# mcychan/nQuant.android

Measured on NVIDIA B200. Metric: Mpixels/s 256-color PNN quantize+dither, 4K batch, 1/2/4/8 B200 vs JVM CPU, higher is better.
Workload: dtype f64

## Files before the change

### include/nquant_b200.h

```cpp
#ifndef NQUANT_B200_H
#define NQUANT_B200_H

#include <stdint.h>

#ifdef __cplusplus
extern "C" {
#endif

#define NQ_KIND_PNN 0
#define NQ_KIND_PNNLAB 1

#define NQ_OK 0
#define NQ_ERR_CUDA (-1)
#define NQ_ERR_ARG (-2)
#define NQ_ERR_COLOR (-3)
#define NQ_ERR_UNSUPPORTED (-4)
#define NQ_ERR_NOMEM (-5)

typedef struct nq_ctx nq_ctx;

int nq_device_count(void);

nq_ctx* nq_create(int device);
void nq_destroy(nq_ctx* ctx);
// ... 24 lines not shown
                           int dither, uint64_t rng_seed, const uint32_t* palette_in, int palette_len, uint32_t* argb_out);

int nq_histogram(nq_ctx* ctx, int kind, const uint32_t* argb_in, int width, int height, int n_max_colors, int* n_bins,
                 double* bins5, float* init_err, int* init_nn, int capacity);

int nq_gilbert_order(int width, int height, uint32_t* order_out);


typedef struct nq_image_info {
  int has_semi_transparency;
  int transparent_pixel_index;
  uint32_t transparent_color;
  int maxbins, quan_rt, texicab, is_nano;
  double weight, ratio_init, ratio_merge, pr, pg, pb, pa;
  int g_margin, g_thresold, g_dither_max_q, g_dither_max, g_sorted, g_has_alpha, g_use_saliency;
  float g_beta;
  float bn_weight;
  int palette_len;
  unsigned long long merges, rescans, pair_tests, rng_draws, heap_pops;
  int error;
  unsigned long long full_evals;
  unsigned long long merge_cycles[6], live_blocks, screened;
  unsigned long long dither_cycles[3];
} nq_image_info;
int nq_get_image_info(nq_ctx* ctx, int image, nq_image_info* out);
int nq_sizeof_image_info(void);

int nq_set_spec_dither(nq_ctx* ctx, int on, int segment, int warmup);
int nq_get_spec_stats(nq_ctx* ctx, unsigned long long* images, unsigned long long* rounds, unsigned long long* fallbacks);

int nq_set_debug(nq_ctx* ctx, int flag);
int nq_debug_get_bins(nq_ctx* ctx, int image, double* bins5, float* init_err, int* init_nn);
int nq_debug_get_merges(nq_ctx* ctx, int image, int* pairs);
int nq_debug_get_saliencies(nq_ctx* ctx, int image, float* out);

unsigned long long nq_kernel_launches(nq_ctx* ctx);
int nq_get_stage_times(nq_ctx* ctx, double* ms, unsigned long long* launches, int reset);
int nq_get_kernel_times(nq_ctx* ctx, double* ms, unsigned long long* launches, int reset);
int nq_debug_math(nq_ctx* ctx, int fn, const double* x, const double* y, double* out, int n);

int nq_debug_ciede(nq_ctx* ctx, const float* lab1, const float* lab2, float* out, int* n_exact, int n);

int nq_synth_device(nq_ctx* ctx, uint32_t* d_out, int n_images, int width, int height, int cls, int alpha_mode,
                    uint64_t seed0);

#ifdef __cplusplus
// ... 4 lines not shown
```

### nquant_android_b200/_lib.py

```python
import ctypes
import os

HERE = os.path.dirname(os.path.abspath(__file__))
SO = os.path.join(HERE, "libnquant_b200.so")

SYMBOLS = [
    "nq_device_count", "nq_create", "nq_destroy", "nq_last_error", "nq_convert", "nq_convert_batch",
    "nq_convert_batch_device", "nq_dither_with_palette", "nq_gilbert_order", "nq_get_image_info", "nq_set_debug",
    "nq_debug_get_bins", "nq_debug_get_merges", "nq_debug_get_saliencies", "nq_kernel_launches", "nq_debug_math",
    "nq_synth_device", "nq_get_stage_times", "nq_set_stream", "nq_debug_ciede", "nq_sizeof_image_info",
    "nq_set_spec_dither", "nq_get_spec_stats", "nq_reset_stream", "nq_set_chunk_images", "nq_get_kernel_times", "nq_convert_batch_multi", "nq_histogram",
]

NQ_KIND_PNN, NQ_KIND_PNNLAB = 0, 1
NQ_OK, NQ_ERR_CUDA, NQ_ERR_ARG, NQ_ERR_COLOR, NQ_ERR_UNSUPPORTED, NQ_ERR_NOMEM = 0, -1, -2, -3, -4, -5


class ImageInfo(ctypes.Structure):
    _fields_ = [
        ("has_semi_transparency", ctypes.c_int), ("transparent_pixel_index", ctypes.c_int),
        ("transparent_color", ctypes.c_uint32),
        ("maxbins", ctypes.c_int), ("quan_rt", ctypes.c_int), ("texicab", ctypes.c_int), ("is_nano", ctypes.c_int),
        ("weight", ctypes.c_double), ("ratio_init", ctypes.c_double), ("ratio_merge", ctypes.c_double),
        ("pr", ctypes.c_double), ("pg", ctypes.c_double), ("pb", ctypes.c_double), ("pa", ctypes.c_double),
        ("g_margin", ctypes.c_int), ("g_thresold", ctypes.c_int), ("g_dither_max_q", ctypes.c_int),
        ("g_dither_max", ctypes.c_int), ("g_sorted", ctypes.c_int), ("g_has_alpha", ctypes.c_int),
        ("g_use_saliency", ctypes.c_int),
        ("g_beta", ctypes.c_float), ("bn_weight", ctypes.c_float), ("palette_len", ctypes.c_int),
        ("merges", ctypes.c_ulonglong), ("rescans", ctypes.c_ulonglong), ("pair_tests", ctypes.c_ulonglong),
        ("rng_draws", ctypes.c_ulonglong), ("heap_pops", ctypes.c_ulonglong),
        ("error", ctypes.c_int),
        ("full_evals", ctypes.c_ulonglong),
        ("merge_cycles", ctypes.c_ulonglong * 6), ("live_blocks", ctypes.c_ulonglong), ("screened", ctypes.c_ulonglong),
        ("dither_cycles", ctypes.c_ulonglong * 3),
    ]

    def as_dict(self):
        return {n: (list(getattr(self, n)) if n in ("merge_cycles", "dither_cycles") else getattr(self, n)) for n, _ in self._fields_}


_lib = None


def load():
    global _lib
    if _lib is not None:
        return _lib
    if not os.path.exists(SO):
        raise ImportError(f"{SO} is missing: run `python -c 'import __graft_entry__ as g; g.build()'` "
                          "(nvcc, sm_100a). This package has no CPU fallback.")
    L = ctypes.CDLL(SO)
    vp, ci, u64 = ctypes.c_void_p, ctypes.c_int, ctypes.c_uint64
    L.nq_device_count.restype = ci
    L.nq_create.restype = vp
    L.nq_create.argtypes = [ci]
    L.nq_destroy.argtypes = [vp]
    L.nq_destroy.restype = None
# ... 32 lines not shown
```

### nquant_android_b200/csrc/nq_api.cu

```cuda
#include <cuda_runtime.h>
#include <stdint.h>
#include <stdio.h>
#include <stdlib.h>
#include <string.h>
#include <string>
#include <vector>
#include <map>
#include <utility>
#include <algorithm>
#include <mutex>
#include <thread>
#include <atomic>
#include <nvtx3/nvToolsExt.h>

#include "../../include/nquant_b200.h"
#include "nq_types.h"
#include "nq_math.h"
#include "nq_color.h"
#include "nq_bluenoise_table.h"
#include "nq_hist.cuh"
#include "nq_pnn.cuh"
#include "nq_dither.cuh"
#include "nq_dither_spec.cuh"

// ... 129 lines not shown
  std::vector<double> bins5;
  std::vector<float> initErr;
  std::vector<int> initNn;
  std::vector<int> merges;
  std::vector<float> sal;
};

}

#define NQ_FRONT_STREAMS 2
#define NQ_SPEC_BULK_DEFAULT 0

struct nq_ctx {
  int device = 0;
  cudaStream_t stream = nullptr;
  cudaStream_t ownStream = nullptr;
  cudaStream_t sFront[NQ_FRONT_STREAMS] = {}, sDith = nullptr, sAux = nullptr, sOut = nullptr, sIn = nullptr;
  std::vector<cudaEvent_t> evPool;
  size_t evUsed = 0;
  int smCount = 148;
  unsigned long long launches = 0;
  bool debug = false;
  int chunkImages = 0;
  int mergeRot = 0;
  std::map<std::pair<int, int>, uint32_t*> orders;
  std::vector<std::pair<int, int>> orderLru;
  size_t orderBytes = 0;
  unsigned char* ws = nullptr;
  size_t wsBytes = 0;
  NqImage* dImgs = nullptr;
  NqSlot* dSlots = nullptr;
  int* dLive = nullptr;
  int* dPos = nullptr;
  unsigned char* zeroPlane = nullptr;
  unsigned char* memoPlane = nullptr;
  unsigned char* sortPool = nullptr;
  size_t zeroSlotBytes = 0, memoSlotBytes = 0, sortSetBytes = 0, sortABytes = 0;
  int wsSlots = 0, wsNpix = 0, wsKind = -1, sortSets = 0;
  bool wsDebug = false, wsBits = false, wsIdx = false;
  std::vector<NqSlot> hSlots;
  uint32_t* dIn = nullptr;
  uint32_t* dOut = nullptr;
  size_t stageBytes = 0;
  double stageMs[NQ_NSTAGES] = {};
  unsigned long long stageLaunches[NQ_NSTAGES] = {};
  double kernelMs[NQ_NKERNELS] = {};
  unsigned long long kernelLaunches[NQ_NKERNELS] = {};
// ... 403 lines not shown
        std::vector<double> col(mb);
        std::vector<float> colf(mb);
        for (int k = 0; k < 4; ++k) {
          if (kind == NQ_KIND_RGB) {
            const double* src = k == 0 ? S.bAc : k == 1 ? S.bC1 : k == 2 ? S.bC2 : S.bC3;
            CU(cudaMemcpy(col.data(), src, (size_t)mb * 8, cudaMemcpyDeviceToHost));
          } else {
            const float* src = k == 0 ? S.fAc : k == 1 ? S.fC1 : k == 2 ? S.fC2 : S.fC3;
            CU(cudaMemcpy(colf.data(), src, (size_t)mb * 4, cudaMemcpyDeviceToHost));
            for (int b = 0; b < mb; ++b) col[b] = colf[b];
          }
          for (int b = 0; b < mb; ++b) D.bins5[(size_t)b * 5 + k] = col[b];
        }
        CU(cudaMemcpy(colf.data(), S.bCnt, (size_t)mb * 4, cudaMemcpyDeviceToHost));
        for (int b = 0; b < mb; ++b) D.bins5[(size_t)b * 5 + 4] = colf[b];
        CU(cudaMemcpy(D.initErr.data(), S.bErr, (size_t)mb * 4, cudaMemcpyDeviceToHost));
        CU(cudaMemcpy(D.initNn.data(), S.bNn, (size_t)mb * 4, cudaMemcpyDeviceToHost));
      }
    }
    if (A.stopAfterSweep) { mark(4); CU(cudaGetLastError()); return NQ_OK; }
    int* live = c->dLive + (size_t)ch.base * NQ_NBINS;
    int* pos = c->dPos + (size_t)ch.base * NQ_NBINS;
    if (kind == NQ_KIND_RGB) {
      nq::k_merge_rgb<<<n, NQ_RGB_THREADS, (size_t)NQ_RGB_HEAP_SMEM * 8, st>>>(dI, dS, live, pos, c->debug ? 1 : 0, c->mergeRot); ++c->launches;
    } else {
      nq::k_merge_lab<<<n, NQ_LAB_THREADS, (size_t)NQ_LAB_HEAP_SMEM * 8, st>>>(dI, dS, live, pos, c->debug ? 1 : 0, c->mergeRot); ++c->launches;
    }
  } else { mark(2); mark(3); }
  mark(4);
  CU(cudaGetLastError());
  return NQ_OK;
}

int run_dither(nq_ctx* c, Chunk& ch, const GroupArgs& A, const uint32_t* dOrder) {
  NvtxRange nv("nq dither (setup, Gilbert pass, BlueNoise pass)");
  const int n = ch.n, npix = A.w * A.h, kind = A.kind;
  cudaStream_t st = c->sDith, ax = c->sAux;
  NqImage* dI = c->dImgs + ch.base;
  NqSlot* dS = c->dSlots + ch.base;
  unsigned long long l0 = c->launches;
  CU(cudaStreamWaitEvent(st, ch.ev[4], 0));
  CU(cudaEventRecord(ch.evD[0], st));
  nq::k_dither_setup<<<(n + 63) / 64, 64, 0, st>>>(dI, dS, n); ++c->launches;
  if (A.dPalIn) {
    for (int i = 0; i < n; ++i) { k_set_palette<<<1, 256, 0, st>>>(dI, i, A.dPalIn, A.palInLen); ++c->launches; }
    nq::k_dither_setup<<<(n + 63) / 64, 64, 0, st>>>(dI, dS, n); ++c->launches;
  }
  const dim3 pg(pixel_grid_x(c, npix, n), n);
  if (kind == NQ_KIND_LAB && c->debug) { nq::k_saliency<<<pg, 256, 0, st>>>(dI, dS); ++c->launches; }
// ... 260 lines not shown
  if (device < 0 || device >= n) { fail(NQ_ERR_CUDA, "no such CUDA device (this library has no CPU fallback)"); return nullptr; }
  if (cudaSetDevice(device) != cudaSuccess) { fail(NQ_ERR_CUDA, "cudaSetDevice failed"); return nullptr; }
  nq_ctx* c = new nq_ctx();
  c->device = device;
  cudaDeviceProp prop;
  if (cudaGetDeviceProperties(&prop, device) == cudaSuccess) c->smCount = prop.multiProcessorCount;
  bool ok = cudaStreamCreateWithFlags(&c->ownStream, cudaStreamNonBlocking) == cudaSuccess;
  for (int k = 0; ok && k < NQ_FRONT_STREAMS; ++k) ok = cudaStreamCreateWithFlags(&c->sFront[k], cudaStreamNonBlocking) == cudaSuccess;
  ok = ok && cudaStreamCreateWithFlags(&c->sDith, cudaStreamNonBlocking) == cudaSuccess;
  ok = ok && cudaStreamCreateWithFlags(&c->sAux, cudaStreamNonBlocking) == cudaSuccess;
  ok = ok && cudaStreamCreateWithFlags(&c->sOut, cudaStreamNonBlocking) == cudaSuccess;
  ok = ok && cudaStreamCreateWithFlags(&c->sIn, cudaStreamNonBlocking) == cudaSuccess;
  if (!ok) { fail(NQ_ERR_CUDA, "cudaStreamCreate failed"); destroy_ctx(c, false); return nullptr; }
  c->stream = c->ownStream;
  if (const char* e = getenv("NQ_SPEC_DITHER")) c->specDither = atoi(e) != 0;
  if (const char* e = getenv("NQ_CHUNK")) c->chunkImages = atoi(e);
  {
    const char* e = getenv("NQ_SPEC_BULK");
    const int bulk = e ? (atoi(e) != 0) : NQ_SPEC_BULK_DEFAULT;
    ok = ok && cudaMemcpyToSymbol(nq::spec::g_specBulk, &bulk, sizeof(bulk)) == cudaSuccess;
  }
  if (const char* e = getenv("NQ_SPEC_SLOTS")) c->specSlotsMax = atoi(e);
  if (const char* e = getenv("NQ_SPEC_POOL_GB")) c->specPoolMaxBytes = (size_t)atoi(e) << 30;
  if (const char* e = getenv("NQ_MERGE_ROT")) c->mergeRot = atoi(e) != 0;
  bool haveLut = false;
  {
    DevBuf dBn, dW;
    ok = dBn.alloc(4096) == cudaSuccess && cudaMemcpy(dBn.p, kBlueNoise, 4096, cudaMemcpyHostToDevice) == cudaSuccess &&
         dW.alloc(sizeof(float) * 3 * (NQ_MAXQ + 3)) == cudaSuccess && cudaMalloc(&c->dTanh, sizeof(float) * 512) == cudaSuccess;
    if (ok) {
      nq::k_init_tables<<<4, 256, 0, c->stream>>>(dBn.as<signed char>()); ++c->launches;
      nq::k_init_rtfac<<<1, 256, 0, c->stream>>>(); ++c->launches;
      k_spec_tables<<<2, 256, 0, c->stream>>>(c->dTanh, dW.as<float>()); ++c->launches;
      ok = cudaMemcpyToSymbolAsync(nq::spec::c_specW, dW.p, sizeof(float) * 3 * (NQ_MAXQ + 3), 0, cudaMemcpyDeviceToDevice, c->stream) == cudaSuccess &&
           cudaStreamSynchronize(c->stream) == cudaSuccess;
    }
  }
  if (ok) {
    std::lock_guard<std::mutex> lk(g_lutMutex);
    LabLutEntry& e = g_lut[device];
    if (!e.ptr) {
      ok = cudaMalloc(&e.ptr, sizeof(float4) << 24) == cudaSuccess;
      if (ok) {
        nq::k_build_lab_lut<<<65536, 256, 0, c->stream>>>(e.ptr); ++c->launches;
        const float4* cp = e.ptr;
        ok = cudaMemcpyToSymbolAsync(nq::g_labLut, &cp, sizeof(cp), 0, cudaMemcpyHostToDevice, c->stream) == cudaSuccess &&
             cudaStreamSynchronize(c->stream) == cudaSuccess;
// ... 128 lines not shown
int nq_gilbert_order(int w, int h, uint32_t* out) {
  if (w <= 0 || h <= 0 || !out) return fail(NQ_ERR_ARG, "bad arguments");
  size_t n = 0;
  gilbert_walk(w, h, [&](int x, int y) { out[n++] = (uint32_t)(x + y * w); });
  return n == (size_t)w * h ? NQ_OK : fail(NQ_ERR_ARG, "gilbert walk size mismatch");
}

int nq_get_image_info(nq_ctx* c, int image, nq_image_info* o) {
  if (!c || !o || image < 0 || image >= (int)c->lastImgs.size()) return fail(NQ_ERR_ARG, "no such image in the last batch");
  const NqImage& I = c->lastImgs[image];
  memset(o, 0, sizeof(*o));
  o->has_semi_transparency = I.hasSemi; o->transparent_pixel_index = I.transIdx; o->transparent_color = I.transColor;
  o->maxbins = I.maxbins; o->quan_rt = I.quan_rt; o->texicab = I.texicab; o->is_nano = I.isNano;
  o->weight = I.weight; o->ratio_init = I.ratio; o->ratio_merge = I.ratioMerge;
  o->pr = I.PR; o->pg = I.PG; o->pb = I.PB; o->pa = I.PA;
  o->g_margin = I.gMargin; o->g_thresold = I.gThresold; o->g_dither_max_q = I.gDitherMaxQ; o->g_dither_max = I.gDitherMax;
  o->g_sorted = I.gSorted; o->g_has_alpha = I.gHasAlpha; o->g_use_saliency = I.gUseSal; o->g_beta = I.gBeta;
  o->bn_weight = I.bnWeight; o->palette_len = I.paletteLen;
  o->merges = (I.nmax > 2 && I.extbins > 0) ? (unsigned long long)I.extbins : 0ULL;
  o->rescans = I.statRescans; o->pair_tests = I.statPairs; o->rng_draws = I.rngDraws; o->heap_pops = I.statHeapPops;
  o->full_evals = I.statFullEvals;
  for (int k = 0; k < 6; ++k) o->merge_cycles[k] = I.statCyc[k];
  o->live_blocks = I.statLiveBlocks; o->screened = I.statScreened;
  for (int k = 0; k < 3; ++k) o->dither_cycles[k] = I.statDither[k];
  o->error = I.error;
  return NQ_OK;
}

int nq_sizeof_image_info(void) { return (int)sizeof(nq_image_info); }

int nq_set_stream(nq_ctx* c, void* stream) {
  if (!c) return fail(NQ_ERR_ARG, "null context");
  c->stream = stream ? reinterpret_cast<cudaStream_t>(stream) : cudaStreamLegacy;
  return NQ_OK;
}
int nq_reset_stream(nq_ctx* c) {
  if (!c) return fail(NQ_ERR_ARG, "null context");
  c->stream = c->ownStream;
  return NQ_OK;
}
int nq_set_chunk_images(nq_ctx* c, int images) {
  if (!c || images < 0) return fail(NQ_ERR_ARG, "bad arguments");
  c->chunkImages = images;
  return NQ_OK;
}

// ... 110 lines not shown
```

### nquant_android_b200/csrc/nq_pnn.cuh

```cuda
#pragma once
#include "nq_types.h"
#include "nq_color.h"
#include "nq_hist.cuh"
#include "nq_fastmath.cuh"

namespace nq {

__device__ const float c_coeffs[3][3] = {{0.299f, 0.587f, 0.114f}, {-0.14713f, -0.28886f, 0.436f}, {0.615f, -0.51499f, -0.10001f}};

struct RgbProbe {
  float n1;
  double wa, wr, wg, wb;
  double PR, PG, PB, PA, ratio;
  int start;
  bool semi;
};

__device__ __forceinline__ RgbProbe rgb_probe(const NqImage& I, const NqSlot& S, int idx) {
  RgbProbe P;
  P.n1 = S.bCnt[idx];
  P.wa = S.bAc[idx]; P.wr = S.bC1[idx]; P.wg = S.bC2[idx]; P.wb = S.bC3[idx];
  P.PR = I.PR; P.PG = I.PG; P.PB = I.PB; P.PA = I.PA; P.ratio = I.ratio;
  P.semi = I.hasSemi != 0;
  P.start = 0;
// ... 351 lines not shown
  __device__ __forceinline__ void sift_down(unsigned idnn1, float e1, int heapN) {
    int l = 1, l2;
    for (; (l2 = l + l) <= heapN; l = l2) {
      float ea, eb = 0.f;
      unsigned ia, ib = 0u;
      if (l2 < HS) {
        ea = sErr[l2]; ia = sIdNn[l2];
        if (l2 < heapN) { eb = sErr[l2 + 1]; ib = sIdNn[l2 + 1]; }
      } else {
        const uint4 ch = *reinterpret_cast<const uint4*>(&gH[l2]);
        ea = __uint_as_float(ch.x); ia = ch.y; eb = __uint_as_float(ch.z); ib = ch.w;
      }
      if (l2 < heapN && ea > eb) { ++l2; ea = eb; ia = ib; }
      if (e1 <= ea) break;
      set(l, ia, ea);
    }
    set(l, idnn1, e1);
  }
};
__device__ __forceinline__ unsigned pack_idnn(int id, int nn) { return (unsigned)id | ((unsigned)nn << 16); }

#define NQ_LAB_THREADS 128
#define NQ_LAB_HEAP_SMEM 5632

__device__ __forceinline__ int block_excl_scan_128(int v, int* total, int* sScan ) {
  const unsigned lane = lane_id(), w = threadIdx.x >> 5;
  int x = v;
#pragma unroll
  for (int o = 1; o < 32; o <<= 1) {
    int y = __shfl_up_sync(0xffffffffu, x, o);
    if (lane >= (unsigned)o) x += y;
  }
  if (lane == 31) sScan[w] = x;
  __syncthreads();
  int base = 0, tot = 0;
#pragma unroll
  for (int k = 0; k < NQ_LAB_THREADS / 32; ++k) { const int c = sScan[k]; if (k < (int)w) base += c; tot += c; }
  *total = tot;
  __syncthreads();
  return base + x - v;
}

__device__ __forceinline__ int rebuild_live_lab(const NqSlot& S, const LabScratch& X, int maxbins, int* live, int* posOf, int* sScan) {
  const int t = threadIdx.x;
  const unsigned lane = lane_id(), w = t >> 5;
  const int W = NQ_LAB_THREADS / 32;
// ... 2 lines not shown
  int c = 0;
  for (int b = b0 + (int)lane; b < b1; b += 32) c += S.bMtm[b] != NQ_DELETED;
  int total, j = block_excl_scan_128(c, &total, sScan);
  j = __shfl_sync(0xffffffffu, j, 0);
  for (int base = b0; base < b1; base += 32) {
    const int b = base + (int)lane;
    const bool alive = b < b1 && S.bMtm[b] != NQ_DELETED;
    const unsigned m = __ballot_sync(0xffffffffu, alive);
    if (alive) {
      const int p = j + __popc(m & ((1u << lane) - 1u));
      live[p] = b; posOf[b] = p;
      X.q[p] = make_float4(S.bCnt[b], S.fC1[b], S.fC2[b], S.fC3[b]);
      X.al[p] = S.fAc[b];
    }
    j += __popc(m);
  }
  __syncthreads();
  const int nblk = (total + 31) >> 5;
  for (int blk = t; blk < nblk; blk += NQ_LAB_THREADS) lab_block_summary(X.q, total, blk, X.bs);
  __syncthreads();
  return total;
}

__global__ void __launch_bounds__(NQ_LAB_THREADS, 4) k_merge_lab(NqImage* imgs, const NqSlot* slots, int* liveBuf, int* posBuf, int logMerges, int rot) {
  extern __shared__ unsigned char smemRaw[];
  float* sErr = reinterpret_cast<float*>(smemRaw);
  unsigned* sId = reinterpret_cast<unsigned*>(smemRaw + (size_t)NQ_LAB_HEAP_SMEM * 4);
  __shared__ int sScan[8];
  __shared__ unsigned sBits[64];
  __shared__ unsigned short sBlk[2048];
  __shared__ unsigned sMaskA[32];
  __shared__ unsigned sMaskB[32];
  __shared__ int sOffA[33], sOffB[33];
  __shared__ double sGs[NQ_LAB_THREADS], sGw[NQ_LAB_THREADS], sF[NQ_LAB_THREADS];
  __shared__ int sPos[NQ_LAB_THREADS];
  __shared__ double sErrCur;
  __shared__ int sNnCur, sAction, sB1, sHeapN, sIter, sNLive;

  const int img = blockIdx.x;
  NqImage& I = imgs[img];
  if (I.kind != NQ_KIND_LAB || I.nmax <= 2 || I.skipPnn) return;
  const NqSlot& S = slots[img];
  const LabScratch X = lab_scratch(S);
  const int t = (int)((threadIdx.x + 32u * (rot ? (blockIdx.x & 3u) : 0u)) & 127u);
  const unsigned lane = lane_id(), w = t >> 5;
  const int W = NQ_LAB_THREADS / 32;
  const int maxbins = I.maxbins, extbins = I.extbins;
  int* live = liveBuf + (size_t)img * NQ_NBINS;
  int* posOf = posBuf + (size_t)img * NQ_NBINS;
  HeapView<NQ_LAB_HEAP_SMEM> H{sErr, sId, S.heap};

  if (w == 0) {
    int heapN = 0;
    for (int base = 0; base < maxbins; base += 32) {
      float e = (base + (int)lane < maxbins) ? S.bErr[base + lane] : 0.f;
      const int nnv = (base + (int)lane < maxbins) ? S.bNn[base + lane] : 0;
      const int cnt = min(32, maxbins - base);
      for (int j = 0; j < cnt; ++j) {
        const float err = __shfl_sync(0xffffffffu, e, j);
        const int nnj = __shfl_sync(0xffffffffu, nnv, j);
        int l = ++heapN, l2;
        for (; l > 1; l = l2) {
          l2 = l >> 1;
          float pe = H.err(l2);
          if (pe <= err) break;
          unsigned pid = H.idnn(l2);
          if (lane == 0) H.set(l, pid, pe);
        }
        if (lane == 0) H.set(l, pack_idnn(base + j, nnj), err);
        __syncwarp();
      }
    }
    if (lane == 0) { sHeapN = heapN; sIter = 0; }
  }
  __syncthreads();
  int liveLen = rebuild_live_lab(S, X, maxbins, live, posOf, sScan);
  int liveAtRebuild = liveLen, iterAtRebuild = 0;
  unsigned long long rescans = 0, pairs = 0, fulls = 0, liveBlocks = 0, screened = 0;
  unsigned pops = 0;
  const double ratioMerge = I.ratioMerge;
  long long cyc[6] = {0, 0, 0, 0, 0, 0};
  long long tk = clock64();
  auto tick = [&](int k) { const long long now = clock64(); cyc[k] += now - tk; tk = now; };

  for (;;) {
    if (t == 0) {
      int action = 0;
      if (sIter >= extbins) action = 2;
      else {
        int heapN = sHeapN;
        for (;;) {
          const unsigned top = H.idnn(1);
          int b1 = (int)(top & 0xFFFFu);
          const int tm = S.bTm[b1], mtm = S.bMtm[b1], nmtm = S.bMtm[top >> 16];
          if (tm >= mtm && nmtm <= tm) { action = 0; sB1 = b1; break; }
          if (mtm == NQ_DELETED) {
            const unsigned last = H.idnn(heapN);
            float e1 = H.err(heapN);
            --heapN;
            ++pops;
            H.sift_down(last, e1, heapN);
            continue;
          }
          action = 1; sB1 = b1;
          break;
        }
        sHeapN = heapN;
      }
      sAction = action;
    }
    if (t < 64) sBits[t] = 0u;
    __syncthreads();
    tick(0);
    const int action = sAction;
    if (action == 2) break;
    const int b1 = sB1;

    if (action == 1) {
      ++rescans;
      const int first = posOf[b1] + 1;
      const LabView V{X.q, X.al, X.bs, liveLen};
      const LabProbe P = lab_probe(I, S, b1, ratioMerge);
      double err = 1e100;
      int nn = -1;
      if (w == 0) {
        const int i = first + (int)lane;
        LabCand c;
        const bool alive = i < liveLen && lab_eval_t<false>(P, V, i, err, &c);
        lab_accept_in_order(alive, c, i, err, nn);
        fulls += i < liveLen;
        if (lane == 0) { sErrCur = err; sNnCur = nn; }
      }
      __syncthreads();
      tick(1);
      err = sErrCur; nn = sNnCur;
      const int stop = first + 32;
      const int blkBeg = stop >> 5, nblk = (liveLen + 31) >> 5;
      for (int blk = blkBeg + t; blk < nblk; blk += NQ_LAB_THREADS)
        if (!lab_block_skip(P, V, blk, err)) atomicOr(&sBits[blk >> 5], 1u << (blk & 31));
      __syncthreads();
      if (w == 0) {
        const unsigned m0 = sBits[2 * lane], m1 = sBits[2 * lane + 1];
        const int c = __popc(m0) + __popc(m1);
        int x = c;
#pragma unroll
        for (int o = 1; o < 32; o <<= 1) { int y = __shfl_up_sync(0xffffffffu, x, o); if (lane >= (unsigned)o) x += y; }
        int at = x - c;
        for (unsigned m = m0; m; m &= m - 1) sBlk[at++] = (unsigned short)(64 * lane + (__ffs(m) - 1));
        for (unsigned m = m1; m; m &= m - 1) sBlk[at++] = (unsigned short)(64 * lane + 32 + (__ffs(m) - 1));
        if (lane == 31) sNLive = x;
      }
      __syncthreads();
      tick(2);
      const int nLive = sNLive;
      liveBlocks += nLive;
      for (int g0 = 0; g0 < nLive; g0 += 32) {
        const int gn = min(32, nLive - g0);
        if (t < 32) { sMaskA[t] = 0u; sMaskB[t] = 0u; }
        __syncthreads();
        for (int r0 = w; r0 < gn; r0 += 4 * W) {
          float4 v[4];
#pragma unroll
          for (int u = 0; u < 4; ++u) {
            const int r = r0 + u * W;
            const int i = r < gn ? ((int)sBlk[g0 + r] << 5) + (int)lane : -1;
            v[u] = (i >= stop && i < liveLen) ? X.q[i] : make_float4(-1.f, 0.f, 0.f, 0.f);
          }
#pragma unroll
          for (int u = 0; u < 4; ++u) {
            const int r = r0 + u * W;
            const unsigned m = __ballot_sync(0xffffffffu, lab_cheap_keep_q(P, v[u], err));
            if (lane == 0 && r < gn) sMaskA[r] = m;
          }
        }
        __syncthreads();
        if (w == 0) {
          const int c = __popc(sMaskA[lane]);
          int x = c;
#pragma unroll
          for (int o = 1; o < 32; o <<= 1) { int y = __shfl_up_sync(0xffffffffu, x, o); if (lane >= (unsigned)o) x += y; }
          sOffA[lane + 1] = x;
          if (lane == 0) sOffA[0] = 0;
        }
        __syncthreads();
        const int totalA = sOffA[32];
        auto posA = [&](int sIdx) {
          int lo = 0, hi = 32;
          while (hi - lo > 1) { const int mid = (lo + hi) >> 1; if (sOffA[mid] <= sIdx) lo = mid; else hi = mid; }
          return ((int)sBlk[g0 + lo] << 5) + (int)__fns(sMaskA[lo], 0, sIdx - sOffA[lo] + 1);
        };
        for (int base = 0; base < totalA; base += NQ_LAB_THREADS) {
          const int sIdx = base + t;
          LabCand dummy;
          const bool keep = sIdx < totalA && lab_eval_t<true>(P, V, posA(sIdx), err, &dummy);
          const unsigned m = __ballot_sync(0xffffffffu, keep);
          if (lane == 0) sMaskB[(base >> 5) + w] = m;
        }
        __syncthreads();
        if (w == 0) {
          const int c = __popc(sMaskB[lane]);
          int x = c;
#pragma unroll
          for (int o = 1; o < 32; o <<= 1) { int y = __shfl_up_sync(0xffffffffu, x, o); if (lane >= (unsigned)o) x += y; }
          sOffB[lane + 1] = x;
          if (lane == 0) sOffB[0] = 0;
        }
        __syncthreads();
        tick(3);
        const int total = sOffB[32];
        screened += total;
        for (int base = 0; base < total; base += NQ_LAB_THREADS) {
          const int uIdx = base + t;
          int pos = -1;
          if (uIdx < total) {
            int lo = 0, hi = 32;
            while (hi - lo > 1) { const int mid = (lo + hi) >> 1; if (sOffB[mid] <= uIdx) lo = mid; else hi = mid; }
            const int sIdx = (lo << 5) + (int)__fns(sMaskB[lo], 0, uIdx - sOffB[lo] + 1);
            const int i = posA(sIdx);
            LabCand c;
            if (lab_eval_t<false>(P, V, i, err, &c)) { pos = i; sGs[t] = c.gs; sGw[t] = c.gw; sF[t] = c.f; }
          }
          sPos[t] = pos;
          fulls += uIdx < total;
          __syncthreads();
          if (w == 0) {
            const int cnt = min(NQ_LAB_THREADS, total - base);
            for (int q = 0; q < cnt; q += 32) {
              const int k = q + (int)lane;
              LabCand c{0, 0, 0};
              int pp = -1;
              if (k < cnt) { pp = sPos[k]; if (pp >= 0) { c.gs = sGs[k]; c.gw = sGw[k]; c.f = sF[k]; } }
              lab_accept_in_order(pp >= 0, c, pp, err, nn);
            }
            if (lane == 0) { sErrCur = err; sNnCur = nn; }
          }
          __syncthreads();
          tick(4);
          err = sErrCur; nn = sNnCur;
        }
      }
      pairs += (unsigned long long)max(0, liveLen - first);
      if (t == 0) {
        float e1 = (float)err;
        const int nnBin = nn < 0 ? 0 : live[nn];
        S.bErr[b1] = e1; S.bNn[b1] = nnBin; S.bTm[b1] = sIter;
        H.sift_down(pack_idnn(b1, nnBin), e1, sHeapN);
      }
      __syncthreads();
      tick(0);
      continue;
    }

    if (t == 0) {
      const int nbI = S.bNn[b1];
      const float n1 = S.bCnt[b1], n2 = S.bCnt[nbI];
      const float d = 1.0f / (n1 + n2);
      const float na = d * (n1 * S.fAc[b1] + n2 * S.fAc[nbI]);
      const float nL = d * (n1 * S.fC1[b1] + n2 * S.fC1[nbI]);
      const float nA = d * (n1 * S.fC2[b1] + n2 * S.fC2[nbI]);
      const float nB = d * (n1 * S.fC3[b1] + n2 * S.fC3[nbI]);
      S.fAc[b1] = na; S.fC1[b1] = nL; S.fC2[b1] = nA; S.fC3[b1] = nB;
      S.bCnt[b1] = n1 + n2;
      const int i = sIter + 1;
      S.bMtm[b1] = i;
      S.bMtm[nbI] = NQ_DELETED;
      const int pt = posOf[b1], pn = posOf[nbI];
      X.q[pt] = make_float4(n1 + n2, nL, nA, nB); X.al[pt] = na;
      X.q[pn].x = -1.f;
      {
        float4 s0 = X.bs[2 * (pt >> 5)], s1 = X.bs[2 * (pt >> 5) + 1];
        s0.y = fminf(s0.y, nL); s0.z = fmaxf(s0.z, nL); s0.w = fmaxf(s0.w, chroma_ub(nA, nB));
        s1.x = fminf(s1.x, nA); s1.y = fmaxf(s1.y, nA); s1.z = fminf(s1.z, nB); s1.w = fmaxf(s1.w, nB);
        X.bs[2 * (pt >> 5)] = s0; X.bs[2 * (pt >> 5) + 1] = s1;
      }
      if (logMerges && S.mergeLog) { S.mergeLog[2 * (i - 1)] = b1; S.mergeLog[2 * (i - 1) + 1] = nbI; }
      sIter = i;
    }
    __syncthreads();
    const int it = sIter;
    if ((it - iterAtRebuild) * 4 > liveAtRebuild) {
      liveLen = rebuild_live_lab(S, X, maxbins, live, posOf, sScan);
      liveAtRebuild = liveLen; iterAtRebuild = it;
    }
    tick(5);
  }

  liveLen = rebuild_live_lab(S, X, maxbins, live, posOf, sScan);
  const int plen = extbins > 0 ? I.nmax : maxbins;
  for (int k = t; k < plen; k += NQ_LAB_THREADS) {
    const int b = live[k];
    uint32_t colr;
    if (!lab2rgb(j2i((double)S.fAc[b]), S.fC1[b], S.fC2[b], S.fC3[b], &colr)) { colr = 0; I.error = 3; }
    I.palette[k] = colr;
  }
  if (t == 0) {
    I.paletteLen = plen;
    I.statRescans = rescans; I.statPairs += pairs; I.statHeapPops = pops;
    for (int k = 0; k < 6; ++k) I.statCyc[k] = (unsigned long long)cyc[k];
    I.statLiveBlocks = liveBlocks; I.statScreened = screened;
  }
  if (fulls) atomicAdd(&I.statFullEvals, fulls);
}


#define NQ_RGB_THREADS 128
#define NQ_RGB_HEAP_SMEM 6144

struct RgbScratch {
  double2* rg;
  double2* bc;
  double* al;
  double *cmin, *lo, *hi;
};
__device__ __forceinline__ RgbScratch rgb_scratch(const NqSlot& S) {
  RgbScratch X;
  X.rg = reinterpret_cast<double2*>(S.hSum);
  X.bc = X.rg + NQ_NBINS;
  double* f = reinterpret_cast<double*>(S.fAc);
  X.al = f;
  X.cmin = f + NQ_NBINS; X.lo = X.cmin + 2048; X.hi = X.lo + 3 * 2048;
  return X;
}

__device__ __forceinline__ double rgb_gate_rec(const RgbProbe& P, const double2 rg, const double2 bc, double al, RgbCand* c) {
  const double n2 = bc.y;
  double nerr2 = ((double)P.n1 * n2) / ((double)P.n1 + n2);
// ... 64 lines not shown
  for (int blk = t; blk < nblk; blk += NQ_RGB_THREADS) rgb_block_summary(X, total, blk);
  __syncthreads();
  return total;
}

__device__ __forceinline__ void rgb_accept_in_order(const RgbProbe& P, double gate, const RgbCand& c, int id, double& err, int& nn, double& errMax) {
  const unsigned lane = lane_id();
  unsigned remaining = 0xffffffffu;
  for (;;) {
    const unsigned m = __ballot_sync(0xffffffffu, gate < err) & remaining;
    if (!m) break;
    const int L = __ffs(m) - 1;
    double e = 0;
    if ((int)lane == L) e = rgb_take(P, c, err);
    err = __shfl_sync(0xffffffffu, e, L);
    nn = __shfl_sync(0xffffffffu, id, L);
    errMax = err > errMax ? err : errMax;
    remaining = (L == 31) ? 0u : ~((2u << L) - 1u);
  }
}

static_assert(NQ_RGB_THREADS == NQ_LAB_THREADS, "block_excl_scan_128 is shared");

__global__ void __launch_bounds__(NQ_RGB_THREADS, 4) k_merge_rgb(NqImage* imgs, const NqSlot* slots, int* liveBuf, int* posBuf, int logMerges, int rot) {
  extern __shared__ unsigned char smemRaw[];
  float* sErr = reinterpret_cast<float*>(smemRaw);
  unsigned* sId = reinterpret_cast<unsigned*>(smemRaw + (size_t)NQ_RGB_HEAP_SMEM * 4);
  __shared__ int sScan[8];
  __shared__ unsigned sBits[64];
  __shared__ unsigned short sBlk[2048];
  __shared__ unsigned sMaskA[32];
  __shared__ int sOffA[33];
  __shared__ double sErrCur, sErrMax;
  __shared__ int sNnCur, sAction, sB1, sHeapN, sIter, sNLive;

  const int img = blockIdx.x;
  NqImage& I = imgs[img];
  if (I.kind != NQ_KIND_RGB || I.nmax <= 2 || I.skipPnn) return;
  const NqSlot& S = slots[img];
  const RgbScratch X = rgb_scratch(S);
  const int t = (int)((threadIdx.x + 32u * (rot ? (blockIdx.x & 3u) : 0u)) & 127u);
  const unsigned lane = lane_id(), w = t >> 5;
  const int W = NQ_RGB_THREADS / 32;
  const int maxbins = I.maxbins, extbins = I.extbins;
  int* live = liveBuf + (size_t)img * NQ_NBINS;
  int* posOf = posBuf + (size_t)img * NQ_NBINS;
  HeapView<NQ_RGB_HEAP_SMEM> H{sErr, sId, S.heap};

  if (w == 0) {
    int heapN = 0;
    for (int base = 0; base < maxbins; base += 32) {
      float e = (base + (int)lane < maxbins) ? S.bErr[base + lane] : 0.f;
      const int nnv = (base + (int)lane < maxbins) ? S.bNn[base + lane] : 0;
      const int cnt = min(32, maxbins - base);
      for (int j = 0; j < cnt; ++j) {
        const float err = __shfl_sync(0xffffffffu, e, j);
        const int nnj = __shfl_sync(0xffffffffu, nnv, j);
        int l = ++heapN, l2;
        for (; l > 1; l = l2) {
          l2 = l >> 1;
          float pe = H.err(l2);
          if (pe <= err) break;
          unsigned pid = H.idnn(l2);
          if (lane == 0) H.set(l, pid, pe);
// ... 259 lines not shown
```

### nquant_android_b200/csrc/nq_types.h

```cpp
#pragma once
#include <stdint.h>

#define NQ_MAXK 256
#define NQ_NBINS 65536
#define NQ_DELETED 0xFFFF
#define NQ_MAXQ 25

enum NqKind { NQ_KIND_RGB = 0, NQ_KIND_LAB = 1 };

struct NqImage {
  int kind, width, height, npix, nmax, dither;
  unsigned long long seed;
  unsigned int semiCount;
  int transIdx;
  int hasSemi;
  uint32_t transColor;
  int fixA0;
  int keyTransp;
  int maxbins, extbins, quan_rt, texicab, isNano, skipPnn;
  double PR, PG, PB, PA, ratio, ratioMerge, weight;
  int paletteLen;
  uint32_t palette[NQ_MAXK];
  int gMargin, gThresold, gDitherMaxQ , gDitherMax, gSorted, gHasAlpha, gUseSal;
  float gBeta;
  double gWeight;
  float gWeights[NQ_MAXQ];
  float gW1[1], gW3[3], gW7[7];
  float bnWeight;
  int error;
  unsigned long long statRescans, statPairs, rngDraws, statFullEvals;
  unsigned int statHeapPops;
  unsigned int distinctColors;
  unsigned long long statCyc[6], statLiveBlocks, statScreened;
  unsigned long long statDither[3];
  int specDone;
  unsigned int nonOpaque;
  int bnParallel;
  int pad1;
};

struct NqSlot {
  const uint32_t* in;
  uint32_t* out;
  unsigned int* hCnt;
  unsigned long long* hSum;
  unsigned int* keyOff;
  uint32_t* sortA;
  uint32_t* sortB;
  unsigned int* warpHist;
  float* sal;
  double* bAc; double* bC1; double* bC2; double* bC3;
  float* fAc; float* fC1; float* fC2; float* fC3;
  float* bCnt; float* bErr;
  int* bNn; int* bTm; int* bMtm;
  uint2* heap;
  int* mergeLog;
// ... 6 lines not shown
```

Measured before the change: 744.3.

## Batch up to four stale-bin rescans per round in LAB PNN merge kernel

```diff
diff --git a/include/nquant_b200.h b/include/nquant_b200.h
--- a/include/nquant_b200.h
+++ b/include/nquant_b200.h
@@ -70,6 +70,7 @@
   unsigned long long full_evals;
   unsigned long long merge_cycles[6], live_blocks, screened;
   unsigned long long dither_cycles[3];
+  unsigned long long merge_rounds, rescans_discarded;
 } nq_image_info;
 int nq_get_image_info(nq_ctx* ctx, int image, nq_image_info* out);
 int nq_sizeof_image_info(void);
diff --git a/nquant_android_b200/_lib.py b/nquant_android_b200/_lib.py
--- a/nquant_android_b200/_lib.py
+++ b/nquant_android_b200/_lib.py
@@ -33,6 +33,7 @@
         ("full_evals", ctypes.c_ulonglong),
         ("merge_cycles", ctypes.c_ulonglong * 6), ("live_blocks", ctypes.c_ulonglong), ("screened", ctypes.c_ulonglong),
         ("dither_cycles", ctypes.c_ulonglong * 3),
+        ("merge_rounds", ctypes.c_ulonglong), ("rescans_discarded", ctypes.c_ulonglong),
     ]
 
     def as_dict(self):
diff --git a/nquant_android_b200/csrc/nq_api.cu b/nquant_android_b200/csrc/nq_api.cu
--- a/nquant_android_b200/csrc/nq_api.cu
+++ b/nquant_android_b200/csrc/nq_api.cu
@@ -175,7 +175,6 @@
   unsigned long long launches = 0;
   bool debug = false;
   int chunkImages = 0;
-  int mergeRot = 0;
   std::map<std::pair<int, int>, uint32_t*> orders;
   std::vector<std::pair<int, int>> orderLru;
   size_t orderBytes = 0;
@@ -625,9 +624,9 @@
     int* live = c->dLive + (size_t)ch.base * NQ_NBINS;
     int* pos = c->dPos + (size_t)ch.base * NQ_NBINS;
     if (kind == NQ_KIND_RGB) {
-      nq::k_merge_rgb<<<n, NQ_RGB_THREADS, (size_t)NQ_RGB_HEAP_SMEM * 8, st>>>(dI, dS, live, pos, c->debug ? 1 : 0, c->mergeRot); ++c->launches;
+      nq::k_merge_rgb<<<n, NQ_RGB_THREADS, (size_t)NQ_RGB_HEAP_SMEM * 8, st>>>(dI, dS, live, pos, c->debug ? 1 : 0); ++c->launches;
     } else {
-      nq::k_merge_lab<<<n, NQ_LAB_THREADS, (size_t)NQ_LAB_HEAP_SMEM * 8, st>>>(dI, dS, live, pos, c->debug ? 1 : 0, c->mergeRot); ++c->launches;
+      nq::k_merge_lab<<<n, NQ_LAB_THREADS, (size_t)NQ_LAB_HEAP_SMEM * 8, st>>>(dI, dS, live, pos, c->debug ? 1 : 0); ++c->launches;
     }
   } else { mark(2); mark(3); }
   mark(4);
@@ -934,7 +933,6 @@
   }
   if (const char* e = getenv("NQ_SPEC_SLOTS")) c->specSlotsMax = atoi(e);
   if (const char* e = getenv("NQ_SPEC_POOL_GB")) c->specPoolMaxBytes = (size_t)atoi(e) << 30;
-  if (const char* e = getenv("NQ_MERGE_ROT")) c->mergeRot = atoi(e) != 0;
   bool haveLut = false;
   {
     DevBuf dBn, dW;
@@ -1109,6 +1107,7 @@
   o->full_evals = I.statFullEvals;
   for (int k = 0; k < 6; ++k) o->merge_cycles[k] = I.statCyc[k];
   o->live_blocks = I.statLiveBlocks; o->screened = I.statScreened;
+  o->merge_rounds = I.statRounds; o->rescans_discarded = I.statDiscarded;
   for (int k = 0; k < 3; ++k) o->dither_cycles[k] = I.statDither[k];
   o->error = I.error;
   return NQ_OK;
diff --git a/nquant_android_b200/csrc/nq_pnn.cuh b/nquant_android_b200/csrc/nq_pnn.cuh
--- a/nquant_android_b200/csrc/nq_pnn.cuh
+++ b/nquant_android_b200/csrc/nq_pnn.cuh
@@ -397,6 +397,7 @@
 
 #define NQ_LAB_THREADS 128
 #define NQ_LAB_HEAP_SMEM 5632
+#define NQ_LAB_ROUND 4
 
 __device__ __forceinline__ int block_excl_scan_128(int v, int* total, int* sScan ) {
   const unsigned lane = lane_id(), w = threadIdx.x >> 5;
@@ -445,33 +446,39 @@
   return total;
 }
 
-__global__ void __launch_bounds__(NQ_LAB_THREADS, 4) k_merge_lab(NqImage* imgs, const NqSlot* slots, int* liveBuf, int* posBuf, int logMerges, int rot) {
+__global__ void __launch_bounds__(NQ_LAB_THREADS, 4) k_merge_lab(NqImage* imgs, const NqSlot* slots, int* liveBuf, int* posBuf, int logMerges) {
+  constexpr int R = NQ_LAB_ROUND;
+  static_assert(R >= 1 && 32 * R <= NQ_LAB_THREADS, "a batch holds 32 blocks of each bin of the round, one per thread");
   extern __shared__ unsigned char smemRaw[];
   float* sErr = reinterpret_cast<float*>(smemRaw);
   unsigned* sId = reinterpret_cast<unsigned*>(smemRaw + (size_t)NQ_LAB_HEAP_SMEM * 4);
   __shared__ int sScan[8];
-  __shared__ unsigned sBits[64];
-  __shared__ unsigned short sBlk[2048];
-  __shared__ unsigned sMaskA[32];
-  __shared__ unsigned sMaskB[32];
-  __shared__ int sOffA[33], sOffB[33];
+  __shared__ unsigned sBits[R][64];
+  __shared__ unsigned short sPre[R][65];
+  __shared__ unsigned short sBat[NQ_LAB_THREADS];
+  __shared__ unsigned sMaskA[NQ_LAB_THREADS];
+  __shared__ unsigned sMaskB[NQ_LAB_THREADS];
+  __shared__ int sOffA[NQ_LAB_THREADS + 1], sOffB[NQ_LAB_THREADS];
   __shared__ double sGs[NQ_LAB_THREADS], sGw[NQ_LAB_THREADS], sF[NQ_LAB_THREADS];
   __shared__ int sPos[NQ_LAB_THREADS];
-  __shared__ double sErrCur;
-  __shared__ int sNnCur, sAction, sB1, sHeapN, sIter, sNLive;
+  __shared__ LabProbe sProbe[R];
+  __shared__ double sErrR[R];
+  __shared__ int sBinR[R], sNnR[R], sFirstR[R];
+  __shared__ int sAction, sB1, sHeapN, sIter, sNRound;
 
   const int img = blockIdx.x;
   NqImage& I = imgs[img];
   if (I.kind != NQ_KIND_LAB || I.nmax <= 2 || I.skipPnn) return;
   const NqSlot& S = slots[img];
   const LabScratch X = lab_scratch(S);
-  const int t = (int)((threadIdx.x + 32u * (rot ? (blockIdx.x & 3u) : 0u)) & 127u);
+  const int t = threadIdx.x;
   const unsigned lane = lane_id(), w = t >> 5;
   const int W = NQ_LAB_THREADS / 32;
   const int maxbins = I.maxbins, extbins = I.extbins;
   int* live = liveBuf + (size_t)img * NQ_NBINS;
   int* posOf = posBuf + (size_t)img * NQ_NBINS;
   HeapView<NQ_LAB_HEAP_SMEM> H{sErr, sId, S.heap};
+  const float4 dead = make_float4(-1.f, 0.f, 0.f, 0.f);
 
   if (w == 0) {
     int heapN = 0;
@@ -494,187 +501,259 @@
         __syncwarp();
       }
     }
-    if (lane == 0) { sHeapN = heapN; sIter = 0; }
+    if (lane == 0) { sHeapN = heapN; sIter = 0; sNRound = 0; }
   }
   __syncthreads();
   int liveLen = rebuild_live_lab(S, X, maxbins, live, posOf, sScan);
   int liveAtRebuild = liveLen, iterAtRebuild = 0;
-  unsigned long long rescans = 0, pairs = 0, fulls = 0, liveBlocks = 0, screened = 0;
+  unsigned long long rescans = 0, pairs = 0, fulls = 0, liveBlocks = 0, screened = 0, rounds = 0, discarded = 0;
   unsigned pops = 0;
+  unsigned used = 0;
   const double ratioMerge = I.ratioMerge;
   long long cyc[6] = {0, 0, 0, 0, 0, 0};
   long long tk = clock64();
   auto tick = [&](int k) { const long long now = clock64(); cyc[k] += now - tk; tk = now; };
 
   for (;;) {
-    if (t == 0) {
-      int action = 0;
-      if (sIter >= extbins) action = 2;
-      else {
-        int heapN = sHeapN;
-        for (;;) {
-          const unsigned top = H.idnn(1);
-          int b1 = (int)(top & 0xFFFFu);
-          const int tm = S.bTm[b1], mtm = S.bMtm[b1], nmtm = S.bMtm[top >> 16];
-          if (tm >= mtm && nmtm <= tm) { action = 0; sB1 = b1; break; }
-          if (mtm == NQ_DELETED) {
-            const unsigned last = H.idnn(heapN);
-            float e1 = H.err(heapN);
-            --heapN;
-            ++pops;
-            H.sift_down(last, e1, heapN);
-            continue;
-          }
-          action = 1; sB1 = b1;
-          break;
-        }
-        sHeapN = heapN;
-      }
-      sAction = action;
-    }
-    if (t < 64) sBits[t] = 0u;
+    if (w == 0) {
+      if (lane == 0) {
+        int action = 0;
+        if (sIter >= extbins) action = 2;
+        else {
+          int heapN = sHeapN;
+          const int nRound = sNRound;
+          for (;;) {
+            const unsigned top = H.idnn(1);
+            const int b1 = (int)(top & 0xFFFFu);
+            const int tm = S.bTm[b1], mtm = S.bMtm[b1], nmtm = S.bMtm[top >> 16];
+            if (tm >= mtm && nmtm <= tm) { action = 0; sB1 = b1; break; }
+            if (mtm == NQ_DELETED) {
+              const unsigned last = H.idnn(heapN);
+              float e1 = H.err(heapN);
+              --heapN;
+              ++pops;
+              H.sift_down(last, e1, heapN);
+              continue;
+            }
+            int j = 0;
+            while (j < nRound && sBinR[j] != b1) ++j;
+            if (j == nRound) { action = 1; break; }
+            const float e1 = (float)sErrR[j];
+            const int nnBin = sNnR[j];
+            S.bErr[b1] = e1; S.bNn[b1] = nnBin; S.bTm[b1] = sIter;
+            H.sift_down(pack_idnn(b1, nnBin), e1, heapN);
+            ++rescans;
+            used |= 1u << j;
+            pairs += (unsigned long long)max(0, liveLen - sFirstR[j]);
+          }
+          sHeapN = heapN;
+          if (action != 2) {
+            discarded += (unsigned long long)__popc(~used & (nRound == 32 ? ~0u : (1u << nRound) - 1u));
+            used = 0;
+            sNRound = 0;
+            rounds += action == 1;
+          }
+        }
+        sAction = action;
+      }
+      __syncwarp();
+      if (sAction == 1) {
+        const int l = 1 + (int)lane;
+        float e = 0.f;
+        int b = 0;
+        bool valid = false, stale = false;
+        if (l <= sHeapN) {
+          const unsigned v = H.idnn(l);
+          e = H.err(l); b = (int)(v & 0xFFFFu);
+          const int tm = S.bTm[b], mtm = S.bMtm[b], nmtm = S.bMtm[v >> 16];
+          valid = tm >= mtm && nmtm <= tm;
+          stale = !valid && mtm != NQ_DELETED;
+        }
+        float ve = valid ? e : INFINITY;
+#pragma unroll
+        for (int o = 16; o; o >>= 1) ve = fminf(ve, __shfl_xor_sync(0xffffffffu, ve, o));
+        const unsigned vm = __ballot_sync(0xffffffffu, valid && e == ve);
+        const int lv = vm ? __ffs(vm) - 1 : 32;
+        const bool cand = stale && (e < ve || (e == ve && (int)lane < lv));
+        const unsigned cm = __ballot_sync(0xffffffffu, cand);
+        int rank = 0;
+#pragma unroll
+        for (int k = 0; k < 32; ++k) {
+          const float ek = __shfl_sync(0xffffffffu, e, k);
+          rank += ((cm >> k) & 1u) && (ek < e || (ek == e && k < (int)lane));
+        }
+        if (cand && rank < R) sBinR[rank] = b;
+        if (lane == 0) sNRound = min(R, __popc(cm));
+      }
+    }
     __syncthreads();
     tick(0);
     const int action = sAction;
     if (action == 2) break;
-    const int b1 = sB1;
 
     if (action == 1) {
-      ++rescans;
-      const int first = posOf[b1] + 1;
+      const int n = sNRound;
       const LabView V{X.q, X.al, X.bs, liveLen};
-      const LabProbe P = lab_probe(I, S, b1, ratioMerge);
-      double err = 1e100;
-      int nn = -1;
-      if (w == 0) {
+      for (int k = t; k < R * 64; k += NQ_LAB_THREADS) (&sBits[0][0])[k] = 0u;
+      for (int j = (int)w; j < n; j += W) {
+        const int b = sBinR[j];
+        const LabProbe P = lab_probe(I, S, b, ratioMerge);
+        const int first = posOf[b] + 1;
+        double err = 1e100;
+        int nn = -1;
         const int i = first + (int)lane;
         LabCand c;
         const bool alive = i < liveLen && lab_eval_t<false>(P, V, i, err, &c);
         lab_accept_in_order(alive, c, i, err, nn);
         fulls += i < liveLen;
-        if (lane == 0) { sErrCur = err; sNnCur = nn; }
+        if (lane == 0) { sProbe[j] = P; sErrR[j] = err; sNnR[j] = nn; sFirstR[j] = first; }
       }
       __syncthreads();
       tick(1);
-      err = sErrCur; nn = sNnCur;
-      const int stop = first + 32;
-      const int blkBeg = stop >> 5, nblk = (liveLen + 31) >> 5;
-      for (int blk = blkBeg + t; blk < nblk; blk += NQ_LAB_THREADS)
-        if (!lab_block_skip(P, V, blk, err)) atomicOr(&sBits[blk >> 5], 1u << (blk & 31));
+      const int nblk = (liveLen + 31) >> 5;
+      {
+        int j = -1, base = 0, beg = 0, cnt = 0;
+        for (int k = t;; k += NQ_LAB_THREADS) {
+          while (k >= base + cnt) {
+            if (++j == n) break;
+            base += cnt;
+            beg = (sFirstR[j] + 32) >> 5;
+            cnt = max(0, nblk - beg);
+          }
+          if (j == n) break;
+          const int blk = beg + (k - base);
+          if (!lab_block_skip(sProbe[j], V, blk, sErrR[j])) atomicOr(&sBits[j][blk >> 5], 1u << (blk & 31));
+        }
+      }
       __syncthreads();
-      if (w == 0) {
-        const unsigned m0 = sBits[2 * lane], m1 = sBits[2 * lane + 1];
-        const int c = __popc(m0) + __popc(m1);
+      for (int j = (int)w; j < n; j += W) {
+        const int c0 = __popc(sBits[j][2 * lane]), c = c0 + __popc(sBits[j][2 * lane + 1]);
         int x = c;
 #pragma unroll
         for (int o = 1; o < 32; o <<= 1) { int y = __shfl_up_sync(0xffffffffu, x, o); if (lane >= (unsigned)o) x += y; }
-        int at = x - c;
-        for (unsigned m = m0; m; m &= m - 1) sBlk[at++] = (unsigned short)(64 * lane + (__ffs(m) - 1));
-        for (unsigned m = m1; m; m &= m - 1) sBlk[at++] = (unsigned short)(64 * lane + 32 + (__ffs(m) - 1));
-        if (lane == 31) sNLive = x;
+        sPre[j][2 * lane] = (unsigned short)(x - c);
+        sPre[j][2 * lane + 1] = (unsigned short)(x - c + c0);
+        if (lane == 31) sPre[j][64] = (unsigned short)x;
       }
       __syncthreads();
       tick(2);
-      const int nLive = sNLive;
-      liveBlocks += nLive;
-      for (int g0 = 0; g0 < nLive; g0 += 32) {
-        const int gn = min(32, nLive - g0);
-        if (t < 32) { sMaskA[t] = 0u; sMaskB[t] = 0u; }
+      int nBatch = 0;
+      for (int j = 0; j < n; ++j) nBatch = max(nBatch, (sPre[j][64] + 31) >> 5);
+      for (int g = 0; g < nBatch; ++g) {
+        int gn = 0;
+        {
+          int jt = -1, rt = 0;
+          for (int j = 0; j < n; ++j) {
+            const int e = min(32, max(0, (int)sPre[j][64] - 32 * g));
+            if (jt < 0 && t < gn + e) { jt = j; rt = 32 * g + t - gn; }
+            gn += e;
+          }
+          if (jt >= 0) {
+            int lo = 0, hi = 64;
+            while (hi - lo > 1) { const int mid = (lo + hi) >> 1; if (sPre[jt][mid] <= rt) lo = mid; else hi = mid; }
+            const int blk = (lo << 5) + (int)__fns(sBits[jt][lo], 0, rt - sPre[jt][lo] + 1);
+            sBat[t] = (unsigned short)((jt << 11) | blk);
+          }
+        }
+        liveBlocks += gn;
+        sMaskA[t] = 0u;
+        sMaskB[t] = 0u;
         __syncthreads();
-        for (int r0 = w; r0 < gn; r0 += 4 * W) {
+        for (int r0 = (int)w; r0 < gn; r0 += 4 * W) {
           float4 v[4];
+          int jr[4];
 #pragma unroll
           for (int u = 0; u < 4; ++u) {
             const int r = r0 + u * W;
-            const int i = r < gn ? ((int)sBlk[g0 + r] << 5) + (int)lane : -1;
-            v[u] = (i >= stop && i < liveLen) ? X.q[i] : make_float4(-1.f, 0.f, 0.f, 0.f);
+            const int e = r < gn ? (int)sBat[r] : 0;
+            jr[u] = e >> 11;
+            const int i = ((e & 2047) << 5) + (int)lane;
+            v[u] = (r < gn && i >= sFirstR[jr[u]] + 32 && i < liveLen) ? X.q[i] : dead;
           }
 #pragma unroll
           for (int u = 0; u < 4; ++u) {
             const int r = r0 + u * W;
-            const unsigned m = __ballot_sync(0xffffffffu, lab_cheap_keep_q(P, v[u], err));
+            const unsigned m = __ballot_sync(0xffffffffu, lab_cheap_keep_q(sProbe[jr[u]], v[u], sErrR[jr[u]]));
             if (lane == 0 && r < gn) sMaskA[r] = m;
           }
         }
         __syncthreads();
-        if (w == 0) {
-          const int c = __popc(sMaskA[lane]);
-          int x = c;
-#pragma unroll
-          for (int o = 1; o < 32; o <<= 1) { int y = __shfl_up_sync(0xffffffffu, x, o); if (lane >= (unsigned)o) x += y; }
-          sOffA[lane + 1] = x;
-          if (lane == 0) sOffA[0] = 0;
-        }
+        int totalA;
+        sOffA[t] = block_excl_scan_128(__popc(sMaskA[t]), &totalA, sScan);
+        if (t == 0) sOffA[NQ_LAB_THREADS] = totalA;
         __syncthreads();
-        const int totalA = sOffA[32];
-        auto posA = [&](int sIdx) {
-          int lo = 0, hi = 32;
+        auto posA = [&](int sIdx, int& j) {
+          int lo = 0, hi = gn;
           while (hi - lo > 1) { const int mid = (lo + hi) >> 1; if (sOffA[mid] <= sIdx) lo = mid; else hi = mid; }
-          return ((int)sBlk[g0 + lo] << 5) + (int)__fns(sMaskA[lo], 0, sIdx - sOffA[lo] + 1);
+          const int e = sBat[lo];
+          j = e >> 11;
+          return ((e & 2047) << 5) + (int)__fns(sMaskA[lo], 0, sIdx - sOffA[lo] + 1);
         };
         for (int base = 0; base < totalA; base += NQ_LAB_THREADS) {
           const int sIdx = base + t;
-          LabCand dummy;
-          const bool keep = sIdx < totalA && lab_eval_t<true>(P, V, posA(sIdx), err, &dummy);
+          bool keep = false;
+          if (sIdx < totalA) {
+            int j;
+            const int i = posA(sIdx, j);
+            LabCand dummy;
+            keep = lab_eval_t<true>(sProbe[j], V, i, sErrR[j], &dummy);
+          }
           const unsigned m = __ballot_sync(0xffffffffu, keep);
           if (lane == 0) sMaskB[(base >> 5) + w] = m;
         }
         __syncthreads();
-        if (w == 0) {
-          const int c = __popc(sMaskB[lane]);
-          int x = c;
-#pragma unroll
-          for (int o = 1; o < 32; o <<= 1) { int y = __shfl_up_sync(0xffffffffu, x, o); if (lane >= (unsigned)o) x += y; }
-          sOffB[lane + 1] = x;
-          if (lane == 0) sOffB[0] = 0;
-        }
+        int total;
+        sOffB[t] = block_excl_scan_128(__popc(sMaskB[t]), &total, sScan);
         __syncthreads();
         tick(3);
-        const int total = sOffB[32];
         screened += total;
+        const int nW = (totalA + 31) >> 5;
         for (int base = 0; base < total; base += NQ_LAB_THREADS) {
           const int uIdx = base + t;
-          int pos = -1;
+          int rec = 0;
           if (uIdx < total) {
-            int lo = 0, hi = 32;
+            int lo = 0, hi = nW;
             while (hi - lo > 1) { const int mid = (lo + hi) >> 1; if (sOffB[mid] <= uIdx) lo = mid; else hi = mid; }
             const int sIdx = (lo << 5) + (int)__fns(sMaskB[lo], 0, uIdx - sOffB[lo] + 1);
-            const int i = posA(sIdx);
+            int j;
+            const int i = posA(sIdx, j);
             LabCand c;
-            if (lab_eval_t<false>(P, V, i, err, &c)) { pos = i; sGs[t] = c.gs; sGw[t] = c.gw; sF[t] = c.f; }
-          }
-          sPos[t] = pos;
+            rec = j << 17;
+            if (lab_eval_t<false>(sProbe[j], V, i, sErrR[j], &c)) { rec |= (1 << 16) | i; sGs[t] = c.gs; sGw[t] = c.gw; sF[t] = c.f; }
+          }
+          sPos[t] = rec;
           fulls += uIdx < total;
           __syncthreads();
           if (w == 0) {
             const int cnt = min(NQ_LAB_THREADS, total - base);
             for (int q = 0; q < cnt; q += 32) {
               const int k = q + (int)lane;
+              const int rk = k < cnt ? sPos[k] : 0;
+              const bool alive = k < cnt && ((rk >> 16) & 1);
+              const int jk = k < cnt ? rk >> 17 : -1;
               LabCand c{0, 0, 0};
-              int pp = -1;
-              if (k < cnt) { pp = sPos[k]; if (pp >= 0) { c.gs = sGs[k]; c.gw = sGw[k]; c.f = sF[k]; } }
-              lab_accept_in_order(pp >= 0, c, pp, err, nn);
+              if (alive) { c.gs = sGs[k]; c.gw = sGw[k]; c.f = sF[k]; }
+              const int j0 = __shfl_sync(0xffffffffu, jk, 0), j1 = __shfl_sync(0xffffffffu, jk, min(31, cnt - 1 - q));
+              for (int j = j0; j <= j1; ++j) {
+                double err = sErrR[j];
+                int nn = sNnR[j];
+                lab_accept_in_order(alive && jk == j, c, rk & 0xFFFF, err, nn);
+                __syncwarp();
+                if (lane == 0) { sErrR[j] = err; sNnR[j] = nn; }
+              }
             }
-            if (lane == 0) { sErrCur = err; sNnCur = nn; }
           }
           __syncthreads();
           tick(4);
-          err = sErrCur; nn = sNnCur;
-        }
-      }
-      pairs += (unsigned long long)max(0, liveLen - first);
-      if (t == 0) {
-        float e1 = (float)err;
-        const int nnBin = nn < 0 ? 0 : live[nn];
-        S.bErr[b1] = e1; S.bNn[b1] = nnBin; S.bTm[b1] = sIter;
-        H.sift_down(pack_idnn(b1, nnBin), e1, sHeapN);
-      }
+        }
+      }
+      if (t < n) { const int nn = sNnR[t]; sNnR[t] = nn < 0 ? 0 : live[nn]; }
       __syncthreads();
-      tick(0);
       continue;
     }
 
     if (t == 0) {
+      const int b1 = sB1;
       const int nbI = S.bNn[b1];
       const float n1 = S.bCnt[b1], n2 = S.bCnt[nbI];
       const float d = 1.0f / (n1 + n2);
@@ -721,10 +800,10 @@
     I.statRescans = rescans; I.statPairs += pairs; I.statHeapPops = pops;
     for (int k = 0; k < 6; ++k) I.statCyc[k] = (unsigned long long)cyc[k];
     I.statLiveBlocks = liveBlocks; I.statScreened = screened;
+    I.statRounds = rounds; I.statDiscarded = discarded;
   }
   if (fulls) atomicAdd(&I.statFullEvals, fulls);
 }
-
 
 #define NQ_RGB_THREADS 128
 #define NQ_RGB_HEAP_SMEM 6144
@@ -835,7 +914,7 @@
 
 static_assert(NQ_RGB_THREADS == NQ_LAB_THREADS, "block_excl_scan_128 is shared");
 
-__global__ void __launch_bounds__(NQ_RGB_THREADS, 4) k_merge_rgb(NqImage* imgs, const NqSlot* slots, int* liveBuf, int* posBuf, int logMerges, int rot) {
+__global__ void __launch_bounds__(NQ_RGB_THREADS, 4) k_merge_rgb(NqImage* imgs, const NqSlot* slots, int* liveBuf, int* posBuf, int logMerges) {
   extern __shared__ unsigned char smemRaw[];
   float* sErr = reinterpret_cast<float*>(smemRaw);
   unsigned* sId = reinterpret_cast<unsigned*>(smemRaw + (size_t)NQ_RGB_HEAP_SMEM * 4);
@@ -852,7 +931,7 @@
   if (I.kind != NQ_KIND_RGB || I.nmax <= 2 || I.skipPnn) return;
   const NqSlot& S = slots[img];
   const RgbScratch X = rgb_scratch(S);
-  const int t = (int)((threadIdx.x + 32u * (rot ? (blockIdx.x & 3u) : 0u)) & 127u);
+  const int t = threadIdx.x;
   const unsigned lane = lane_id(), w = t >> 5;
   const int W = NQ_RGB_THREADS / 32;
   const int maxbins = I.maxbins, extbins = I.extbins;
diff --git a/nquant_android_b200/csrc/nq_types.h b/nquant_android_b200/csrc/nq_types.h
--- a/nquant_android_b200/csrc/nq_types.h
+++ b/nquant_android_b200/csrc/nq_types.h
@@ -32,6 +32,7 @@
   unsigned int statHeapPops;
   unsigned int distinctColors;
   unsigned long long statCyc[6], statLiveBlocks, statScreened;
+  unsigned long long statRounds, statDiscarded;
   unsigned long long statDither[3];
   int specDone;
   unsigned int nonOpaque;
```

Result: faster. 793.5 (median of 6 runs) (+6.6%).
